# ZhengmaoHe/PARC

Hardware: AMD Instinct MI355X
Metric: env-steps/sec (whole node), 4096 envs/GPU humanoid tracker at 1/2/4/8 MI355X (higher is better)
Workload: dtype f32; 1 GPU; 4096 envs/GPU tracker on procgen box heightfields, 64 synthetic clips (BASELINE.json configs[2]); envs_per_gpu=4096, env_steps_per_bench_step=131072, rollout_steps=32, update_epochs=5, minibatch=16384, sim_substeps=4, parallelism=dp1, scaling_rule=per-rank work fixed (T = 32, minibatch = 4 x envs): weak scaling, grad_allreduce=per minibatch (reference cadence)

## Files before the change

include/parc_hip.h:

```cpp
#ifndef PARC_HIP_H
#define PARC_HIP_H

#include <stdint.h>

#ifdef __cplusplus
extern "C" {
#endif

#define PARC_MAX_BODIES 16
#define PARC_MAX_DOFS 64
#define PARC_MAX_TAR_STEPS 6
#define PARC_MAX_KEY_BODIES 8

#define PARC_OK 0
#define PARC_EINVAL (-1)
#define PARC_EUNSUPPORTED (-2)

#define PARC_JOINT_ROOT 0
#define PARC_JOINT_HINGE 1
#define PARC_JOINT_SPHERICAL 2
#define PARC_JOINT_FIXED 3

#define PARC_DONE_NULL 0
#define PARC_DONE_FAIL 1
// ... 199 lines not shown

int64_t parc_moments_workspace_floats(int64_t rows, int dim);
int parc_moments_accumulate(void *stream, int64_t rows, int dim, const float *x, float *acc, float *workspace);
int parc_obs_ingest(void *stream, int64_t rows, int dim, const float *x, const float *mean, const float *stdv, float clip, float *norm_out,
                    float *copy_dst, const int64_t *copy_row, float *acc, float *workspace);

int parc_action_head(void *stream, int n, int A, const float *mean, const float *logstd, const float *noise, const float *explore,
                     const float *a_mean, const float *a_std, float *action, float *logp);
int parc_action_head_record(void *stream, int n, int A, const float *mean, const float *logstd, const float *noise, const float *explore,
                            const float *a_mean, const float *a_std, float *action, float *logp, float *rec_action, float *rec_logp,
                            float *rec_mask, const float *forces_src, float *rec_forces, int n_forces, const int64_t *head);

int parc_points_hf_sdf(void *stream, int batch, int n_points, int dim_x, int dim_y, const float *points, const float *hf,
                       const float *min_box_center, const float *x_points, const float *y_points, float half_x, float half_y,
                       float base_z, int inverted, float radius, float *out, int32_t *out_cell);

int parc_points_hf_sdf_grad(void *stream, int batch, int n_points, int dim_x, int dim_y, const float *points, const float *hf,
                            const float *min_box_center, const float *x_points, const float *y_points, float half_x, float half_y,
                            float base_z, int inverted, const int32_t *cell, const float *g_out, float *g_points);

int64_t parc_relu_bwd_workspace_floats(int64_t rows, int dim);
int parc_relu_bwd_bias_grad(void *stream, int64_t rows, int dim, float *gy, const float *y, float *db, float *workspace);
int parc_weighted_colsum(void *stream, int64_t rows, int dim, const float *x, const float *w, float *out, float *workspace);

int parc_abi_version(void);

#ifdef __cplusplus
}
#endif
#endif
```

parc_amd/_hip.py:

```python
import ctypes
import os
import subprocess

import torch

_HERE = os.path.dirname(os.path.abspath(__file__))
LIB_DIR = os.path.join(_HERE, "lib")
LIB_PATH = os.path.join(LIB_DIR, "libparc_hip.so")
CSRC = os.path.join(_HERE, "csrc")
SOURCES = ["parc_kin.hip", "parc_sim.hip", "parc_ppo.hip", "parc_terrain.hip", "parc_render.hip", "parc_score.hip", "parc_netstats.hip", "parc_moopt.hip"]
DIAG_LIB_PATH = os.path.join(LIB_DIR, "libparc_hip_diag.so")
DIAG_SOURCES = SOURCES + ["parc_sim_ref.hip"]

MAX_BODIES = 16
MAX_DOFS = 64
MAX_TAR_STEPS = 6
MAX_KEY_BODIES = 8

POST_REF = 1
POST_OBS = 2
POST_REWARD_DONE = 4
POST_HF = 8
POST_MASKED = 16
POST_INIT_CHAR = 32
# ... 175 lines not shown
    L.parc_ppo_workspace_floats.restype = c_int
    L.parc_normalize_clamp.argtypes = [c_vp, c_i64, c_int, c_vp, c_vp, c_vp, c_f, c_vp]
    L.parc_normalize_clamp.restype = c_int
    L.parc_action_head.argtypes = [c_vp, c_int, c_int] + [c_vp] * 8
    L.parc_action_head.restype = c_int
    L.parc_action_head_record.argtypes = [c_vp, c_int, c_int] + [c_vp] * 8 + [c_vp] * 5 + [c_int, c_vp]
    L.parc_action_head_record.restype = c_int
    L.parc_points_hf_sdf.argtypes = [c_vp, c_int, c_int, c_int, c_int] + [c_vp] * 5 + [c_f, c_f, c_f, c_int, c_f, c_vp, c_vp]
    L.parc_points_hf_sdf.restype = c_int
    L.parc_points_hf_sdf_grad.argtypes = [c_vp, c_int, c_int, c_int, c_int] + [c_vp] * 5 + [c_f, c_f, c_f, c_int, c_vp, c_vp, c_vp]
    L.parc_points_hf_sdf_grad.restype = c_int
    L.parc_scale_by_clipped_norm.argtypes = [c_vp, c_i64, c_vp, c_vp, c_f]
    L.parc_scale_by_clipped_norm.restype = c_int
    L.parc_moments_workspace_floats.argtypes = [c_i64, c_int]
    L.parc_moments_workspace_floats.restype = c_i64
    L.parc_moments_accumulate.argtypes = [c_vp, c_i64, c_int, c_vp, c_vp, c_vp]
    L.parc_moments_accumulate.restype = c_int
    L.parc_relu_bwd_workspace_floats.argtypes = [c_i64, c_int]
    L.parc_relu_bwd_workspace_floats.restype = c_i64
    L.parc_relu_bwd_bias_grad.argtypes = [c_vp, c_i64, c_int, c_vp, c_vp, c_vp, c_vp]
    L.parc_relu_bwd_bias_grad.restype = c_int
    L.parc_weighted_colsum.argtypes = [c_vp, c_i64, c_int, c_vp, c_vp, c_vp, c_vp]
    L.parc_weighted_colsum.restype = c_int
    L.parc_sgd_workspace_floats.argtypes = []
    L.parc_sgd_workspace_floats.restype = c_i64
    L.parc_sgd_momentum_step.argtypes = [c_vp, c_i64, c_vp, c_vp, c_vp, c_f, c_f, c_f, c_f, c_vp, c_vp]
    L.parc_sgd_momentum_step.restype = c_int
    L.parc_adamw_step.argtypes = [c_vp, c_i64, c_vp, c_vp, c_vp, c_vp, c_i64, c_f, c_f, c_f, c_f, c_f, c_f, c_vp, c_vp]
    L.parc_adamw_step.restype = c_int
    L.parc_return_tracker_update.argtypes = [c_vp, c_int, c_int, c_vp, c_i64] + [c_vp] * 8
    L.parc_return_tracker_workspace_floats.argtypes = [c_int]
    L.parc_return_tracker_workspace_floats.restype = c_i64
    L.parc_return_tracker_update.restype = c_int
    L.parc_record_step.argtypes = [c_vp, c_int, c_vp, c_int, c_vp]
    L.parc_record_step.restype = c_int
    L.parc_obs_ingest.argtypes = [c_vp, c_i64, c_int, c_vp, c_vp, c_vp, c_f, c_vp, c_vp, c_vp, c_vp, c_vp]
    L.parc_obs_ingest.restype = c_int
    L.parc_rng_step.argtypes = [c_vp, ctypes.c_uint64, c_vp, c_vp, c_i64, c_vp, c_i64, c_vp, c_int]
    L.parc_rng_step.restype = c_int
    L.parc_reset_apply.argtypes = [c_vp, c_int, c_vp, c_vp, c_vp, c_vp, c_vp, c_int] + [c_vp] * 9
    L.parc_reset_apply.restype = c_int
    L.parc_reset_sample_apply.argtypes = [c_vp, c_int, c_vp, c_vp, c_vp, c_int, c_vp, c_vp, c_f, c_vp, c_vp, c_int, c_f] + [c_vp] * 11
    L.parc_reset_sample_apply.restype = c_int
    for name in ("parc_refresh_ray_obs_hfs", "parc_refresh_obs_hfs", "parc_dof_to_rot", "parc_rot_to_dof",
                 "parc_forward_kinematics", "parc_calc_motion_frame", "parc_motion_lib_build", "parc_track_post_step", "parc_reset_apply",
                 "parc_update_fail_rates", "parc_td_lambda_return", "parc_adv_normalize"):
# ... 6 lines not shown
        _hip_render.declare(L)
    if hasattr(L, "parc_score_abi"):
        from . import _hip_score
        _hip_score.declare(L)
    if hasattr(L, "parc_netstats_abi"):
        from . import _hip_netstats
        _hip_netstats.declare(L)
    if hasattr(L, "parc_moopt_abi"):
        from . import _hip_moopt
        _hip_moopt.declare(L)


EXPORTED = ["parc_abi_version", "parc_refresh_ray_obs_hfs", "parc_refresh_obs_hfs", "parc_dof_to_rot", "parc_rot_to_dof",
            "parc_forward_kinematics", "parc_calc_motion_frame", "parc_motion_lib_build", "parc_track_post_step",
            "parc_update_fail_rates", "parc_td_lambda_return", "parc_adv_normalize", "parc_reset_apply", "parc_ppo_loss", "parc_ppo_workspace_floats", "parc_record_step", "parc_return_tracker_update", "parc_normalize_clamp",
            "parc_action_head", "parc_points_hf_sdf", "parc_moments_workspace_floats", "parc_moments_accumulate", "parc_reset_sample_apply", "parc_return_tracker_workspace_floats", "parc_scale_by_clipped_norm", "parc_relu_bwd_workspace_floats",
            "parc_relu_bwd_bias_grad", "parc_ppo_loss_packed", "parc_weighted_colsum", "parc_sgd_workspace_floats", "parc_sgd_momentum_step", "parc_adamw_step",
            "parc_pose_chain_forward", "parc_pose_chain_backward", "parc_points_hf_sdf_grad", "parc_body_points_world", "parc_body_points_world_grad",
            "parc_quat_diff_angle", "parc_quat_diff_angle_grad", "parc_temporal_terms", "parc_temporal_terms_grad", "parc_step_tail",
            "parc_assemble_obs", "parc_track_post_step_timed", "parc_rng_step", "parc_obs_ingest", "parc_action_head_record",
            "parc_render", "parc_render_abi", "parc_motion_score", "parc_score_abi",
            "parc_netstats_workspace_floats", "parc_netstats_update", "parc_netstats_abs_colsum", "parc_netstats_dormant_count", "parc_netstats_abi",
            "parc_points_hf_sdf_ragged", "parc_points_hf_sdf_ragged_grad", "parc_temporal_terms_seg", "parc_temporal_terms_seg_grad",
            "parc_segment_sums", "parc_moopt_abi"]


def check(rc, what):
    if rc != 0:
        raise RuntimeError("{} failed with code {} ({})".format(what, rc, "bad argument" if rc == -1 else "unsupported" if rc == -2 else "hipError"))


def stream():
    return c_vp(torch.cuda.current_stream().cuda_stream)


def ptr(t):
    if t is None:
        return c_vp(0)
    assert t.is_cuda, "HIP kernels need device tensors (no CPU fallback)"
    assert t.is_contiguous(), "tensor must be contiguous"
    return c_vp(t.data_ptr())


def terrain_struct(hf, min_point, dxdy):
    assert hf.dtype == torch.float32 and hf.is_contiguous() and hf.dim() == 2
    return TerrainS(ptr(hf), int(hf.shape[0]), int(hf.shape[1]), float(min_point[0]), float(min_point[1]),
                    float(dxdy[0]), float(dxdy[1]))
# ... 29 lines not shown
```

parc_amd/csrc/parc_ppo.hip:

```cpp
#include <hip/hip_runtime.h>
#include <math.h>
#include <stdint.h>
#include <stdio.h>
#include <stdlib.h>

#include "../../include/parc_hip.h"

#define PPO_THREADS 256
#define PPO_MAX_A 64
#define PPO_NSCAL 8
#define PPO_W (PPO_NSCAL + PPO_MAX_A)

__device__ __forceinline__ float wave_sum(float v) {
#pragma unroll
    for (int o = 32; o >= 1; o >>= 1) v += __shfl_xor(v, o, 64);
    return v;
}

__device__ __forceinline__ float clamp_nan(float v, float lo, float hi) { return v < lo ? lo : (v > hi ? hi : v); }
__device__ __forceinline__ float clamp_min_nan(float v, float lo) { return v < lo ? lo : v; }
__device__ __forceinline__ float clamp_max_nan(float v, float hi) { return v > hi ? hi : v; }
__device__ __forceinline__ float minimum_nan(float a, float b) { return a <= b ? a : (b < a ? b : __builtin_nanf("")); }
__device__ __forceinline__ float clip_coef(float max_norm, float norm) { return clamp_max_nan(max_norm / (norm + 1e-6f), 1.0f); }

// ... 184 lines not shown
        out[0] = actor_loss + cfg.critic_w * critic_loss;
        out[1] = critic_loss;
        out[2] = actor_loss;
        out[3] = s[3] / cnt;
        out[4] = s[4] / cnt;
        out[5] = abl;
        out[6] = ent;
        out[7] = regl;
        out[8] = cnt;
        out[9] = gate / cnt;
        out[10] = cfg.critic_w / (float)B;
    }
}

__global__ __launch_bounds__(256) void ppo_scale_kernel(int n_mean, int n_pred, const float *__restrict__ out, float *g_mean, float *g_pred) {
    const int i = blockIdx.x * blockDim.x + threadIdx.x;
    const float sa = out[9], sp = out[10];
    if (i < n_mean) g_mean[i] *= sa;
    if (i < n_pred) g_pred[i] *= sp;
}

static int ppo_loss_impl(void *stream, int B, int A, const float *mean, const float *logstd, const float *norm_a, const float *old_logp,
                         const float *adv, const float *mask, const float *pred, const float *tar_val, parc_ppo_cfg_t cfg, float *g_mean,
                         float *g_logstd, float *g_pred, float *out, float *workspace, int a_stride, int s_stride);

extern "C" int parc_ppo_loss(void *stream, int B, int A, const float *mean, const float *logstd, const float *norm_a, const float *old_logp,
                             const float *adv, const float *mask, const float *pred, const float *tar_val, parc_ppo_cfg_t cfg, float *g_mean,
                             float *g_logstd, float *g_pred, float *out, float *workspace) {
    return ppo_loss_impl(stream, B, A, mean, logstd, norm_a, old_logp, adv, mask, pred, tar_val, cfg, g_mean, g_logstd, g_pred, out, workspace, A, 1);
}

extern "C" int parc_ppo_loss_packed(void *stream, int B, int A, const float *mean, const float *logstd, const float *rec, int rec_stride,
                                    const float *pred, parc_ppo_cfg_t cfg, float *g_mean, float *g_logstd, float *g_pred, float *out,
                                    float *workspace) {
    if (!rec || rec_stride < A + 4) return PARC_EINVAL;
    return ppo_loss_impl(stream, B, A, mean, logstd, rec, rec + A, rec + A + 1, rec + A + 2, pred, rec + A + 3, cfg, g_mean, g_logstd, g_pred, out,
                         workspace, rec_stride, rec_stride);
}

static int ppo_loss_impl(void *stream, int B, int A, const float *mean, const float *logstd, const float *norm_a, const float *old_logp,
                         const float *adv, const float *mask, const float *pred, const float *tar_val, parc_ppo_cfg_t cfg, float *g_mean,
                         float *g_logstd, float *g_pred, float *out, float *workspace, int a_stride, int s_stride) {
    if (B <= 0 || A <= 0 || A > PPO_MAX_A) return PARC_EINVAL;
    int nblk = (B + PPO_THREADS - 1) / PPO_THREADS;
    hipStream_t st = (hipStream_t)stream;
    if (A <= 32) {
        nblk = (B + PPO32_SPB - 1) / PPO32_SPB;
        hipLaunchKernelGGL(ppo_sample32_kernel, dim3(nblk), dim3(256), 0, st, B, A, mean, logstd, norm_a, old_logp, adv, mask, pred, tar_val, cfg,
                           g_mean, g_pred, workspace, a_stride, s_stride);
    } else {
        hipLaunchKernelGGL(ppo_sample_kernel, dim3(nblk), dim3(PPO_THREADS), 0, st, B, A, mean, logstd, norm_a, old_logp, adv, mask, pred, tar_val,
                           cfg, g_mean, g_pred, workspace, a_stride, s_stride);
    }
    hipLaunchKernelGGL(ppo_reduce_kernel, dim3(1), dim3(PPO_RED_THREADS), 0, st, B, A, nblk, logstd, cfg, workspace, g_logstd, out);
    const int n = B * A;
    hipLaunchKernelGGL(ppo_scale_kernel, dim3((n + 255) / 256), dim3(256), 0, st, n, B, out, g_mean, g_pred);
    hipError_t e = hipGetLastError();
    return e == hipSuccess ? PARC_OK : (int)e;
}

extern "C" int parc_ppo_workspace_floats(int B) { return ((B + PPO32_SPB - 1) / PPO32_SPB) * PPO_W; }

#define PARC_RECORD_MAX_FIELDS 12
struct record_fields_t {
    parc_record_field_t f[PARC_RECORD_MAX_FIELDS];
};

__global__ __launch_bounds__(256) void record_step_kernel(int n_envs, const int64_t *__restrict__ head, record_fields_t fields) {
    const parc_record_field_t f = fields.f[blockIdx.y];
    const size_t total = (size_t)n_envs * (size_t)f.row_bytes;
    const size_t h = (size_t)head[0];
    const size_t tid = (size_t)blockIdx.x * blockDim.x + threadIdx.x, nthr = (size_t)gridDim.x * blockDim.x;
    if (f.convert == 1) {
        const int64_t *s = (const int64_t *)f.src;
        int32_t *d = (int32_t *)f.dst + h * (total / 8);
        for (size_t i = tid; i < total / 8; i += nthr) d[i] = (int32_t)s[i];
        return;
    }
    if (f.convert == 2) {
// ... 574 lines not shown
    hipLaunchKernelGGL(colsum_final_kernel, dim3((dim + 255) / 256), dim3(256), 0, (hipStream_t)stream, chunks, dim, workspace, out);
    hipError_t e = hipGetLastError();
    return e == hipSuccess ? PARC_OK : (int)e;
}

extern "C" int64_t parc_relu_bwd_workspace_floats(int64_t rows, int dim) {
    if (rows < 0 || dim <= 0) return -1;
    return ((rows + RB_ROWS - 1) / RB_ROWS) * (int64_t)dim;
}

extern "C" int parc_relu_bwd_bias_grad(void *stream, int64_t rows, int dim, float *gy, const float *y, float *db, float *workspace) {
    if (rows < 0 || dim <= 0 || (dim & 3) || !gy || !y || !db || !workspace || (((uintptr_t)gy | (uintptr_t)y | (uintptr_t)workspace) & 15))
        return PARC_EINVAL;
    if (rows > (int64_t)RB_ROWS * 65535) return PARC_EUNSUPPORTED;
    const int dim4 = dim / 4, chunks = (int)((rows + RB_ROWS - 1) / RB_ROWS);
    if (rows > 0)
        hipLaunchKernelGGL(relu_bwd_bias_partial_kernel, dim3((dim4 + 63) / 64, chunks), dim3(256), 0, (hipStream_t)stream, (int)rows, dim4,
                           (float4 *)gy, (const float4 *)y, (float4 *)workspace);
    hipLaunchKernelGGL(colsum_final_kernel, dim3((dim + 255) / 256), dim3(256), 0, (hipStream_t)stream, chunks, dim, workspace, db);
    hipError_t e = hipGetLastError();
    return e == hipSuccess ? PARC_OK : (int)e;
}

__global__ __launch_bounds__(256) void action_head_kernel(int n, int A, const float *__restrict__ mean, const float *__restrict__ logstd,
                                                          const float *__restrict__ noise, const float *__restrict__ explore,
                                                          const float *__restrict__ a_mean, const float *__restrict__ a_std, float *action,
                                                          float *logp) {
    const int i = blockIdx.x * blockDim.x + threadIdx.x;
    if (i >= n) return;
    const bool ex = explore[i] == 1.0f;
    float acc = 0.f, sum_ls = 0.f;
    for (int j = 0; j < A; ++j) {
        const float ls = logstd[j], sd = __expf(ls);
        const float mu = mean[(size_t)i * A + j];
        const float na = ex ? mu + sd * noise[(size_t)i * A + j] : mu;
        const float z = (na - mu) / sd;
        acc = fmaf(z, z, acc);
        sum_ls += ls;
        action[(size_t)i * A + j] = na * a_std[j] + a_mean[j];
    }
    logp[i] = -0.5f * acc + (-0.5f * (float)A * 1.8378770664093453f - sum_ls);
}

struct action_record_t {
    float *action, *logp, *mask, *forces;
    const float *forces_src;
// ... 73 lines not shown
```

parc_amd/learning/dm_ppo_agent.py:

```python
import enum
import os
import time

import numpy as np
import torch

from ..envs import base_env
from ..gym_spaces import Box
from ..util import mp_util
from ..util.logger import Logger
from . import dm_ppo_model, experience_buffer, mp_optimizer, normalizer, rl_util, unit_stats
from .dm_ppo_return_tracker import DMPPOReturnTracker
from .tracking_error_tracker import TrackingErrorTracker


class AgentMode(enum.Enum):
    TRAIN = 0
    TEST = 1


_LOSS_KEYS = ["norm_obs", "action", "a_logp", "tar_val", "adv", "rand_action_mask"]


def enable_tuned_gemms():
# ... 466 lines not shown
                        "test_mean_body_rot_tracking_err": t.get_mean_body_rot_err().item(),
                        "test_mean_dof_vel_tracking_err": t.get_mean_dof_vel_err().item(),
                        "test_mean_root_vel_tracking_err": t.get_mean_root_vel_err().item(),
                        "test_mean_root_ang_vel_tracking_err": t.get_mean_root_ang_vel_err().item()})
        return out

    def hard_reset_envs(self):
        if self._is_terrain_runner:
            self._env.apply_hard_reset()
        self._curr_obs, self._curr_info = self._env.reset()

    def test_model(self, num_episodes):
        self.eval()
        self.set_mode(AgentMode.TEST)
        self.hard_reset_envs()
        P = mp_util.get_num_procs()
        return self._rollout_test(int(np.ceil(num_episodes / P)))

    @torch.no_grad()
    def _critic_values(self):
        eb = self._exp_buffer
        obs, next_obs, done = eb.get_data("obs"), eb.get_data("next_obs"), eb.get_data("done")
        norm_obs = self._obs_norm.normalize(obs, out=eb.get_data("norm_obs"))
        vals = self._model.eval_critic(norm_obs).squeeze(-1)
        T = obs.shape[0]
        need = done != base_env.DoneFlags.NULL.value
        need[T - 1] = True
        next_vals = torch.empty_like(vals)
        next_vals[:T - 1] = vals[1:]
        idx = need.flatten().nonzero().flatten()
        sel = next_obs.flatten(0, 1)[idx]
        next_vals.flatten()[idx] = self._model.eval_critic(self._obs_norm.normalize(sel)).squeeze(-1)
        return vals, next_vals

    @torch.no_grad()
    def _build_train_data(self):
        self.eval()
        eb = self._exp_buffer
        obs, next_obs = eb.get_data("obs"), eb.get_data("next_obs")
        r, done = eb.get_data("reward"), eb.get_data("done")
        mask = eb.get_data("rand_action_mask")
        vals, next_vals = self._critic_values()
        r_min, r_max = self._env.get_reward_bounds()
        next_vals = torch.clamp(next_vals, r_min / (1.0 - self._discount), r_max / (1.0 - self._discount))
        succ_val = self._env.get_reward_succ() / (1.0 - self._discount)
        fail_val = self._env.get_reward_fail() / (1.0 - self._discount)
        next_vals = torch.where(done == base_env.DoneFlags.SUCC.value, torch.full_like(next_vals, succ_val), next_vals)
        next_vals = torch.where(done == base_env.DoneFlags.FAIL.value, torch.full_like(next_vals, fail_val), next_vals)
# ... 60 lines not shown
            return None
        loss, out = rl_util.ppo_loss(a_dist.mean, logstd[0], pred, norm_a, batch["a_logp"], batch["adv"], batch["rand_action_mask"],
                                     batch["tar_val"], self._ppo_clip_ratio, self._action_bound_weight, self._action_entropy_weight,
                                     self._action_reg_weight, self._critic_loss_weight, 20.0, self._critic_loss_type != "L2")
        slots = {"loss": 0, "critic_loss": 1, "actor_loss": 2, "clip_frac": 3, "imp_ratio": 4}
        if self._action_bound_weight != 0:
            slots["action_bound_loss"] = 5
        if self._action_entropy_weight != 0:
            slots["action_entropy"] = 6
        if self._action_reg_weight != 0:
            slots["action_reg_loss"] = 7
        return {"loss": loss, "_packed": out, "_slots": slots}

    def _explicit_update_ok(self):
        return (str(self._device).startswith("cuda") and self._config.get("explicit_backward", True) and self._config.get("fused_ppo_loss", True)
                and self._model.supports_explicit_backward())

    def _minibatch_step_explicit(self, batch, acc):
        norm_obs = batch["norm_obs"]
        mean, logstd, pred, saved = self._model.train_forward(norm_obs)
        if self._ppo_cfg is None:
            self._ppo_cfg = rl_util.ppo_cfg(self._ppo_clip_ratio, self._action_bound_weight, self._action_entropy_weight, self._action_reg_weight,
                                            self._critic_loss_weight, 20.0, self._critic_loss_type != "L2")
        if "loss_rec" in batch:
            out, g_mean, g_logstd, g_pred = rl_util.ppo_loss_and_grads_packed(mean, logstd, pred, batch["loss_rec"], self._ppo_cfg)
        else:
            out, g_mean, g_logstd, g_pred = rl_util.ppo_loss_and_grads(mean, logstd, pred, self._a_norm.normalize(batch["action"]), batch["a_logp"],
                                                                        batch["adv"], batch["rand_action_mask"], batch["tar_val"], self._ppo_cfg)
        write = lambda grad_of, done: self._model.train_backward(saved, g_mean, g_logstd, g_pred, grad_of, done)
        if self._clip_grad_norm:
            self._optimizer.step_explicit(write, model=self._model, max_norm=self._max_grad_norm)
        else:
            self._optimizer.step_explicit(write)
        acc.append(out)

    def _nan_trap(self, loss_rows, batches, epoch):
        bad = torch.isnan(loss_rows).any(dim=1).tolist()
        if not any(bad):
            return
        k = bad.index(True)
        import pickle
        batch_file = os.path.join("output", "debug_batch.pkl")
        os.makedirs("output", exist_ok=True)
        with open(batch_file, "wb") as f:
            pickle.dump({name: v.detach().cpu() for name, v in batches[k].items()}, f)
        Logger.print("NAN LOSS in minibatch {} of update epoch {}: wrote debug batch file to {}".format(k, epoch, batch_file))
        raise FloatingPointError("NaN loss in minibatch {} of update epoch {} (batch dumped to {}; the reference prints, dumps and exits "
                                 "at this point)".format(k, epoch, batch_file))

    def _update_model(self):
        self.train()
        N = self.get_num_envs()
# ... 196 lines not shown
```

parc_amd/learning/dm_ppo_model.py:

```python
import enum

import numpy as np
import torch


class StdType(enum.Enum):
    FIXED = 0
    CONSTANT = 1
    VARIABLE = 2


class DistributionGaussianDiag:
    def __init__(self, mean, logstd):
        self._mean = mean
        self._logstd = logstd
        self._std_cache = None
        self._dim = mean.shape[-1]

    @property
    def _std(self):
        if self._std_cache is None:
            self._std_cache = torch.exp(self._logstd)
        return self._std_cache

# ... 156 lines not shown
        pred = torch.addmm(self._critic_out.bias, c[-1], self._critic_out.weight.t()).squeeze(-1)
        return mean, self._action_dist._logstd_net, pred, (a, c)

    def _relu_bwd(self, d, y, db):
        from .. import _hip
        L = _hip.lib()
        need = int(L.parc_relu_bwd_workspace_floats(d.shape[0], d.shape[1]))
        ws = getattr(self, "_relu_ws", None)
        if ws is None or ws.numel() < need or ws.device != d.device:
            ws = self._relu_ws = torch.empty(max(need, 1), dtype=torch.float32, device=d.device)
        _hip.check(L.parc_relu_bwd_bias_grad(_hip.stream(), d.shape[0], d.shape[1], _hip.ptr(d), _hip.ptr(y), _hip.ptr(db), _hip.ptr(ws)),
                   "parc_relu_bwd_bias_grad")

    def _weighted_colsum(self, x, w, out):
        from .. import _hip
        L = _hip.lib()
        need = int(L.parc_relu_bwd_workspace_floats(x.shape[0], x.shape[1]))
        ws = getattr(self, "_relu_ws", None)
        if ws is None or ws.numel() < need or ws.device != x.device:
            ws = self._relu_ws = torch.empty(max(need, 1), dtype=torch.float32, device=x.device)
        _hip.check(L.parc_weighted_colsum(_hip.stream(), x.shape[0], x.shape[1], _hip.ptr(x), _hip.ptr(w.contiguous()), _hip.ptr(out), _hip.ptr(ws)),
                   "parc_weighted_colsum")

    def _trunk_backward(self, seq, acts, d, grad_of, done):
        lins = list(seq)[0::2]
        for k in range(len(lins) - 1, -1, -1):
            lin = lins[k]
            self._relu_bwd(d, acts[k + 1], grad_of(lin.bias))
            torch.mm(d.t(), acts[k], out=grad_of(lin.weight))
            done(lin.weight)
            done(lin.bias)
            if k > 0:
                d = torch.mm(d, lin.weight)

    @torch.no_grad()
    def train_backward(self, saved, g_mean, g_logstd, g_pred, grad_of, done=lambda p: None):
        a, c = saved
        mnet = self._action_dist._mean_net
        torch.mm(g_mean.t(), a[-1], out=grad_of(mnet.weight))
        torch.sum(g_mean, dim=0, out=grad_of(mnet.bias))
        done(mnet.weight)
        done(mnet.bias)
        if self._action_dist._std_type == StdType.CONSTANT:
            grad_of(self._action_dist._logstd_net).copy_(g_logstd)
            done(self._action_dist._logstd_net)
        self._trunk_backward(self._actor_layers, a, torch.mm(g_mean, mnet.weight), grad_of, done)
        gp = g_pred.unsqueeze(-1)
        if self._critic_out.weight.shape[0] == 1:
            self._weighted_colsum(c[-1], g_pred, grad_of(self._critic_out.weight).view(-1))
        else:
            torch.mm(gp.t(), c[-1], out=grad_of(self._critic_out.weight))
        torch.sum(gp, dim=0, out=grad_of(self._critic_out.bias))
        done(self._critic_out.weight)
        done(self._critic_out.bias)
        self._trunk_backward(self._critic_layers, c, torch.mm(gp, self._critic_out.weight), grad_of, done)

    def eval_critic(self, obs):
        return self._critic_out(self._critic_layers(obs))
```

parc_amd/learning/rl_util.py:

```python
import torch

from .. import _hip

_workspace = {}


def compute_td_lambda_return(r, next_vals, done, discount, td_lambda):
    assert r.shape == next_vals.shape and r.dim() == 2
    r = r.contiguous().float()
    nv = next_vals.contiguous().float()
    dn = done.contiguous().to(torch.int32)
    T, N = r.shape
    ret = torch.empty_like(r)
    _hip.check(_hip.lib().parc_td_lambda_return(_hip.stream(), T, N, _hip.ptr(r), _hip.ptr(nv), _hip.ptr(dn), float(discount),
                                                float(td_lambda), _hip.ptr(ret)), "parc_td_lambda_return")
    return ret


def normalize_advantage(ret, vals, rand_action_mask, clip):
    ret = ret.contiguous().float()
    vals = vals.contiguous().float()
    mask = rand_action_mask.contiguous().float()
    dev = ret.device
    ws = _workspace.get(dev)
    if ws is None:
        ws = torch.empty(3 * 1024, dtype=torch.float64, device=dev)
        _workspace[dev] = ws
    out = torch.empty_like(ret)
    ms = torch.empty(2, dtype=torch.float32, device=dev)
    _hip.check(_hip.lib().parc_adv_normalize(_hip.stream(), ret.numel(), _hip.ptr(ret), _hip.ptr(vals), _hip.ptr(mask), float(clip),
                                             _hip.ptr(out), _hip.ptr(ms), _hip.ptr(ws)), "parc_adv_normalize")
    return out, ms


def ppo_loss_and_grads(mean, logstd, pred, norm_a, old_logp, adv, mask, tar_val, cfg):
    from .. import _hip
    B, A = mean.shape
    mean, norm_a = mean.contiguous(), norm_a.contiguous()
    g_mean = torch.empty_like(mean)
    g_logstd = torch.empty_like(logstd)
    g_pred = torch.empty(B, dtype=torch.float32, device=mean.device)
    out = torch.empty(16, dtype=torch.float32, device=mean.device)
    ws = torch.empty(_hip.lib().parc_ppo_workspace_floats(B), dtype=torch.float32, device=mean.device)
    p = _hip.ptr
    _hip.check(_hip.lib().parc_ppo_loss(_hip.stream(), B, A, p(mean), p(logstd.contiguous()), p(norm_a), p(old_logp.contiguous()),
                                        p(adv.contiguous()), p(mask.contiguous()), p(pred.contiguous()), p(tar_val.contiguous()), cfg,
                                        p(g_mean), p(g_logstd), p(g_pred), p(out), p(ws)), "parc_ppo_loss")
    return out, g_mean, g_logstd, g_pred


def ppo_loss_and_grads_packed(mean, logstd, pred, rec, cfg):
    from .. import _hip
    B, A = mean.shape
    assert rec.dim() == 2 and rec.shape[0] == B and rec.shape[1] >= A + 4 and rec.is_contiguous()
    mean = mean.contiguous()
    g_mean = torch.empty_like(mean)
    g_logstd = torch.empty_like(logstd)
    g_pred = torch.empty(B, dtype=torch.float32, device=mean.device)
    out = torch.empty(16, dtype=torch.float32, device=mean.device)
    ws = torch.empty(_hip.lib().parc_ppo_workspace_floats(B), dtype=torch.float32, device=mean.device)
    p = _hip.ptr
    _hip.check(_hip.lib().parc_ppo_loss_packed(_hip.stream(), B, A, p(mean), p(logstd.contiguous()), p(rec), int(rec.shape[1]), p(pred.contiguous()),
                                               cfg, p(g_mean), p(g_logstd), p(g_pred), p(out), p(ws)), "parc_ppo_loss_packed")
    return out, g_mean, g_logstd, g_pred


def ppo_cfg(clip_ratio, bound_w, entropy_w, reg_w, critic_w, large_critic_loss=20.0, critic_l1=False):
    from .. import _hip
    return _hip.PPOCfgS(float(clip_ratio), float(bound_w), float(entropy_w), float(reg_w), float(critic_w), float(large_critic_loss),
                        int(bool(critic_l1)))


class _PPOLossFn(torch.autograd.Function):

    @staticmethod
    def forward(ctx, mean, logstd, pred, norm_a, old_logp, adv, mask, tar_val, cfg):
        out, g_mean, g_logstd, g_pred = ppo_loss_and_grads(mean, logstd, pred, norm_a, old_logp, adv, mask, tar_val, cfg)
        ctx.save_for_backward(g_mean, g_logstd, g_pred)
        ctx.mark_non_differentiable(out)
        return out[0], out

    @staticmethod
    def backward(ctx, g_loss, _g_out):
        g_mean, g_logstd, g_pred = ctx.saved_tensors
        return g_mean * g_loss, g_logstd * g_loss, g_pred * g_loss, None, None, None, None, None, None

# ... 6 lines not shown
```

Measured before the change: 454,400 env-steps/s.

## Fuse output-head backward with ReLU mask, bias and weight gradients

Adds a HIP head-backward kernel that computes the output-layer weight and bias gradients, the propagated gradient through the head weights, the ReLU mask, and the last hidden layer's bias gradient in one pass over the activations. The default critic path (J=1) now uses it instead of separate weighted-colsum, matmul and relu-bwd launches. An optional mode skips the PPO loss scale kernel and folds the loss scales into the head backward, but it is disabled by default. The aim is fewer kernel launches and fewer reads of the large activation tensor in the minibatch backward. The cost is extra code paths and a reduction order that differs from before.

```diff
diff --git a/include/parc_hip.h b/include/parc_hip.h
--- a/include/parc_hip.h
+++ b/include/parc_hip.h
@@ -245,6 +245,15 @@
 int64_t parc_relu_bwd_workspace_floats(int64_t rows, int dim);
 int parc_relu_bwd_bias_grad(void *stream, int64_t rows, int dim, float *gy, const float *y, float *db, float *workspace);
 int parc_weighted_colsum(void *stream, int64_t rows, int dim, const float *x, const float *w, float *out, float *workspace);
+int64_t parc_head_bwd_workspace_floats(int64_t rows, int h, int J);
+int parc_head_bwd(void *stream, int64_t rows, int h, int J, const float *Wh, const float *g, const float *scale, const float *y, float *d,
+                  float *db, float *dWh, float *dbh, float *workspace);
+int parc_ppo_loss_unscaled(void *stream, int B, int A, const float *mean, const float *logstd, const float *norm_a, const float *old_logp,
+                           const float *adv, const float *mask, const float *pred, const float *tar_val, parc_ppo_cfg_t cfg, float *g_mean,
+                           float *g_logstd, float *g_pred, float *out, float *workspace);
+int parc_ppo_loss_packed_unscaled(void *stream, int B, int A, const float *mean, const float *logstd, const float *rec, int rec_stride,
+                                  const float *pred, parc_ppo_cfg_t cfg, float *g_mean, float *g_logstd, float *g_pred, float *out,
+                                  float *workspace);
 
 int parc_abi_version(void);
 
diff --git a/parc_amd/_hip.py b/parc_amd/_hip.py
--- a/parc_amd/_hip.py
+++ b/parc_amd/_hip.py
@@ -221,6 +221,14 @@
     L.parc_relu_bwd_bias_grad.restype = c_int
     L.parc_weighted_colsum.argtypes = [c_vp, c_i64, c_int, c_vp, c_vp, c_vp, c_vp]
     L.parc_weighted_colsum.restype = c_int
+    L.parc_head_bwd_workspace_floats.argtypes = [c_i64, c_int, c_int]
+    L.parc_head_bwd_workspace_floats.restype = c_i64
+    L.parc_head_bwd.argtypes = [c_vp, c_i64, c_int, c_int] + [c_vp] * 9
+    L.parc_head_bwd.restype = c_int
+    L.parc_ppo_loss_unscaled.argtypes = L.parc_ppo_loss.argtypes
+    L.parc_ppo_loss_unscaled.restype = c_int
+    L.parc_ppo_loss_packed_unscaled.argtypes = L.parc_ppo_loss_packed.argtypes
+    L.parc_ppo_loss_packed_unscaled.restype = c_int
     L.parc_sgd_workspace_floats.argtypes = []
     L.parc_sgd_workspace_floats.restype = c_i64
     L.parc_sgd_momentum_step.argtypes = [c_vp, c_i64, c_vp, c_vp, c_vp, c_f, c_f, c_f, c_f, c_vp, c_vp]
@@ -273,7 +281,8 @@
             "parc_render", "parc_render_abi", "parc_motion_score", "parc_score_abi",
             "parc_netstats_workspace_floats", "parc_netstats_update", "parc_netstats_abs_colsum", "parc_netstats_dormant_count", "parc_netstats_abi",
             "parc_points_hf_sdf_ragged", "parc_points_hf_sdf_ragged_grad", "parc_temporal_terms_seg", "parc_temporal_terms_seg_grad",
-            "parc_segment_sums", "parc_moopt_abi"]
+            "parc_segment_sums", "parc_moopt_abi",
+            "parc_head_bwd_workspace_floats", "parc_head_bwd", "parc_ppo_loss_unscaled", "parc_ppo_loss_packed_unscaled"]
 
 
 def check(rc, what):
diff --git a/parc_amd/csrc/parc_ppo.hip b/parc_amd/csrc/parc_ppo.hip
--- a/parc_amd/csrc/parc_ppo.hip
+++ b/parc_amd/csrc/parc_ppo.hip
@@ -230,7 +230,7 @@
 
 static int ppo_loss_impl(void *stream, int B, int A, const float *mean, const float *logstd, const float *norm_a, const float *old_logp,
                          const float *adv, const float *mask, const float *pred, const float *tar_val, parc_ppo_cfg_t cfg, float *g_mean,
-                         float *g_logstd, float *g_pred, float *out, float *workspace, int a_stride, int s_stride);
+                         float *g_logstd, float *g_pred, float *out, float *workspace, int a_stride, int s_stride, bool apply_scale = true);
 
 extern "C" int parc_ppo_loss(void *stream, int B, int A, const float *mean, const float *logstd, const float *norm_a, const float *old_logp,
                              const float *adv, const float *mask, const float *pred, const float *tar_val, parc_ppo_cfg_t cfg, float *g_mean,
@@ -246,9 +246,24 @@
                          workspace, rec_stride, rec_stride);
 }
 
+extern "C" int parc_ppo_loss_unscaled(void *stream, int B, int A, const float *mean, const float *logstd, const float *norm_a, const float *old_logp,
+                                      const float *adv, const float *mask, const float *pred, const float *tar_val, parc_ppo_cfg_t cfg,
+                                      float *g_mean, float *g_logstd, float *g_pred, float *out, float *workspace) {
+    return ppo_loss_impl(stream, B, A, mean, logstd, norm_a, old_logp, adv, mask, pred, tar_val, cfg, g_mean, g_logstd, g_pred, out, workspace, A, 1,
+                         false);
+}
+
+extern "C" int parc_ppo_loss_packed_unscaled(void *stream, int B, int A, const float *mean, const float *logstd, const float *rec, int rec_stride,
+                                             const float *pred, parc_ppo_cfg_t cfg, float *g_mean, float *g_logstd, float *g_pred, float *out,
+                                             float *workspace) {
+    if (!rec || rec_stride < A + 4) return PARC_EINVAL;
+    return ppo_loss_impl(stream, B, A, mean, logstd, rec, rec + A, rec + A + 1, rec + A + 2, pred, rec + A + 3, cfg, g_mean, g_logstd, g_pred, out,
+                         workspace, rec_stride, rec_stride, false);
+}
+
 static int ppo_loss_impl(void *stream, int B, int A, const float *mean, const float *logstd, const float *norm_a, const float *old_logp,
                          const float *adv, const float *mask, const float *pred, const float *tar_val, parc_ppo_cfg_t cfg, float *g_mean,
-                         float *g_logstd, float *g_pred, float *out, float *workspace, int a_stride, int s_stride) {
+                         float *g_logstd, float *g_pred, float *out, float *workspace, int a_stride, int s_stride, bool apply_scale) {
     if (B <= 0 || A <= 0 || A > PPO_MAX_A) return PARC_EINVAL;
     int nblk = (B + PPO_THREADS - 1) / PPO_THREADS;
     hipStream_t st = (hipStream_t)stream;
@@ -262,7 +277,7 @@
     }
     hipLaunchKernelGGL(ppo_reduce_kernel, dim3(1), dim3(PPO_RED_THREADS), 0, st, B, A, nblk, logstd, cfg, workspace, g_logstd, out);
     const int n = B * A;
-    hipLaunchKernelGGL(ppo_scale_kernel, dim3((n + 255) / 256), dim3(256), 0, st, n, B, out, g_mean, g_pred);
+    if (apply_scale) hipLaunchKernelGGL(ppo_scale_kernel, dim3((n + 255) / 256), dim3(256), 0, st, n, B, out, g_mean, g_pred);
     hipError_t e = hipGetLastError();
     return e == hipSuccess ? PARC_OK : (int)e;
 }
@@ -883,6 +898,256 @@
     return e == hipSuccess ? PARC_OK : (int)e;
 }
 
+#define HB_ROWS 64
+#define HB_COLS 512
+template <int JP, int NS>
+__global__ __launch_bounds__(256 * NS) void head_bwd_partial_kernel(int rows, int h, int J, const float *__restrict__ Wh, const float *__restrict__ g,
+                                                                    const float *__restrict__ scale, const float *__restrict__ y,
+                                                                    float *__restrict__ d, float *__restrict__ partial) {
+    constexpr int HB_U = JP >= 16 ? 4 : 8;
+    constexpr int GR = HB_ROWS / NS;
+    constexpr int NV = 2 * JP + 2;
+    __shared__ __attribute__((aligned(16))) float s_g[HB_ROWS * JP];
+    __shared__ float s_fold[(NS - 1) * NV * 256];
+    const int tid = threadIdx.x & 255, grp = threadIdx.x >> 8;
+    const int r0 = blockIdx.y * HB_ROWS, nr = min(HB_ROWS, rows - r0);
+    const int c0 = blockIdx.x * HB_COLS + tid, c1 = c0 + 256;
+    const bool v0 = c0 < h, v1 = c1 < h;
+    const int cc0 = v0 ? c0 : 0, cc1 = v1 ? c1 : 0;
+    const float sc = scale ? scale[0] : 1.f;
+    for (int i = threadIdx.x; i < HB_ROWS * JP; i += 256 * NS) {
+        const int r = i / JP, j = i - r * JP;
+        float v = 0.f;
+        if (r < nr && j < J) {
+            v = g[(size_t)(r0 + r) * J + j];
+            if (scale) v *= sc;
+        }
+        s_g[i] = v;
+    }
+    float w0[JP], w1[JP], a0[JP], a1[JP];
+#pragma unroll
+    for (int j = 0; j < JP; ++j) {
+        w0[j] = j < J ? Wh[(size_t)j * h + cc0] : 0.f;
+        w1[j] = j < J ? Wh[(size_t)j * h + cc1] : 0.f;
+        a0[j] = 0.f;
+        a1[j] = 0.f;
+    }
+    float b0 = 0.f, b1 = 0.f;
+    const int g0 = grp * GR, ge = min(g0 + GR, nr);
+    const float *yb = y + (size_t)r0 * h;
+    float *dr = d + (size_t)r0 * h;
+    float n0[HB_U], n1[HB_U];
+#pragma unroll
+    for (int u = 0; u < HB_U; ++u) {
+        const int r = min(g0 + u, nr - 1);
+        n0[u] = yb[(size_t)r * h + cc0];
+        n1[u] = yb[(size_t)r * h + cc1];
+    }
+    __syncthreads();
+    for (int rb = g0; rb < ge; rb += HB_U) {
+        float y0[HB_U], y1[HB_U];
+#pragma unroll
+        for (int u = 0; u < HB_U; ++u) {
+            y0[u] = n0[u];
+            y1[u] = n1[u];
+        }
+#pragma unroll
+        for (int u = 0; u < HB_U; ++u) {
+            const int r = min(rb + HB_U + u, nr - 1);
+            n0[u] = yb[(size_t)r * h + cc0];
+            n1[u] = yb[(size_t)r * h + cc1];
+        }
+#pragma unroll
+        for (int u = 0; u < HB_U; ++u) {
+            const int r = rb + u;
+            if (r < ge) {
+                const float *gr = s_g + r * JP;
+                float s0 = 0.f, s1 = 0.f;
+#pragma unroll
+                for (int j = 0; j < JP; ++j) {
+                    const float gj = gr[j];
+                    s0 = fmaf(gj, w0[j], s0);
+                    s1 = fmaf(gj, w1[j], s1);
+                    a0[j] = fmaf(gj, y0[u], a0[j]);
+                    a1[j] = fmaf(gj, y1[u], a1[j]);
+                }
+                const float d0 = y0[u] <= 0.f ? 0.f : s0, d1 = y1[u] <= 0.f ? 0.f : s1;
+                if (v0) dr[(size_t)r * h + c0] = d0;
+                if (v1) dr[(size_t)r * h + c1] = d1;
+                b0 += d0;
+                b1 += d1;
+            }
+        }
+    }
+    if (grp > 0) {
+        float *f = s_fold + (size_t)(grp - 1) * NV * 256 + tid;
+#pragma unroll
+        for (int j = 0; j < JP; ++j) {
+            f[(2 * j) * 256] = a0[j];
+            f[(2 * j + 1) * 256] = a1[j];
+        }
+        f[(2 * JP) * 256] = b0;
+        f[(2 * JP + 1) * 256] = b1;
+    }
+    __syncthreads();
+    if (grp > 0) return;
+#pragma unroll
+    for (int s = 0; s < NS - 1; ++s) {
+        const float *f = s_fold + (size_t)s * NV * 256 + tid;
+#pragma unroll
+        for (int j = 0; j < JP; ++j) {
+            a0[j] += f[(2 * j) * 256];
+            a1[j] += f[(2 * j + 1) * 256];
+        }
+        b0 += f[(2 * JP) * 256];
+        b1 += f[(2 * JP + 1) * 256];
+    }
+    float *p = partial + (size_t)blockIdx.y * ((size_t)J * h + h + J);
+#pragma unroll
+    for (int j = 0; j < JP; ++j) {
+        if (j < J) {
+            if (v0) p[(size_t)j * h + c0] = a0[j];
+            if (v1) p[(size_t)j * h + c1] = a1[j];
+        }
+    }
+    if (v0) p[(size_t)J * h + c0] = b0;
+    if (v1) p[(size_t)J * h + c1] = b1;
+    if (blockIdx.x == 0 && tid < J) {
+        float t = 0.f;
+        for (int r = 0; r < nr; ++r) t += s_g[r * JP + tid];
+        p[(size_t)J * h + h + tid] = t;
+    }
+}
+
+template <int P>
+__global__ __launch_bounds__(256) void head_bwd_final_kernel(int chunks, int h, int J, const float *__restrict__ partial, float *__restrict__ dWh,
+                                                             float *__restrict__ db, float *__restrict__ dbh) {
+    constexpr int E = 256 / P;
+    __shared__ float sp[P][E];
+    const int lane = threadIdx.x % E, part = threadIdx.x / E;
+    const int n = J * h + h + J, e = blockIdx.x * E + lane;
+    const int per = (chunks + P - 1) / P, k0 = part * per, k1 = min(k0 + per, chunks);
+    float t = 0.f;
+    if (e < n) {
+#pragma unroll 16
+        for (int k = k0; k < k1; ++k) t += partial[(size_t)k * n + e];
+    }
+    sp[part][lane] = t;
+    __syncthreads();
+    if (part == 0 && e < n) {
+        float v = sp[0][lane];
+#pragma unroll
+        for (int q = 1; q < P; ++q) v += sp[q][lane];
+        if (e < J * h) dWh[e] = v;
+        else if (e < J * h + h) db[e - J * h] = v;
+        else dbh[e - J * h - h] = v;
+    }
+}
+
+__global__ __launch_bounds__(256) void head1_bwd_partial_kernel(int rows, int dim4, const float4 *__restrict__ wh, const float *__restrict__ g,
+                                                                const float *__restrict__ scale, const float4 *__restrict__ y,
+                                                                float4 *__restrict__ d, float4 *__restrict__ partial, float *__restrict__ pbh) {
+    __shared__ float4 red[2][4][64];
+    const int lane = threadIdx.x & 63, rg = threadIdx.x >> 6;
+    const int c = blockIdx.x * 64 + lane;
+    const int r0 = blockIdx.y * RB_ROWS, r1 = min(r0 + RB_ROWS, rows);
+    const float sc = scale ? scale[0] : 1.f;
+    float4 s = make_float4(0.f, 0.f, 0.f, 0.f), t = s;
+    if (c < dim4) {
+        const float4 w = wh[c];
+#pragma unroll 4
+        for (int r = r0 + rg; r < r1; r += 4) {
+            const size_t i = (size_t)r * dim4 + c;
+            const float4 v = y[i];
+            float gr = g[r];
+            if (scale) gr *= sc;
+            s.x = fmaf(gr, v.x, s.x); s.y = fmaf(gr, v.y, s.y); s.z = fmaf(gr, v.z, s.z); s.w = fmaf(gr, v.w, s.w);
+            float4 o;
+            o.x = v.x <= 0.f ? 0.f : __fmul_rn(gr, w.x); o.y = v.y <= 0.f ? 0.f : __fmul_rn(gr, w.y);
+            o.z = v.z <= 0.f ? 0.f : __fmul_rn(gr, w.z); o.w = v.w <= 0.f ? 0.f : __fmul_rn(gr, w.w);
+            d[i] = o;
+            t.x += o.x; t.y += o.y; t.z += o.z; t.w += o.w;
+        }
+    }
+    red[0][rg][lane] = s;
+    red[1][rg][lane] = t;
+    __syncthreads();
+    if (rg < 2 && c < dim4) {
+        const float4 a = red[rg][0][lane], b = red[rg][1][lane], e = red[rg][2][lane], f = red[rg][3][lane];
+        float4 o;
+        o.x = (a.x + b.x) + (e.x + f.x); o.y = (a.y + b.y) + (e.y + f.y); o.z = (a.z + b.z) + (e.z + f.z); o.w = (a.w + b.w) + (e.w + f.w);
+        partial[((size_t)blockIdx.y * 2 + rg) * dim4 + c] = o;
+    }
+    if (pbh && blockIdx.x == 0 && threadIdx.x == 0) {
+        float b = 0.f;
+        for (int r = r0; r < r1; ++r) {
+            float gr = g[r];
+            if (scale) gr *= sc;
+            b += gr;
+        }
+        pbh[blockIdx.y] = b;
+    }
+}
+
+__global__ __launch_bounds__(256) void head1_bwd_final_kernel(int chunks, int dim, const float *__restrict__ partial, const float *__restrict__ pbh,
+                                                              float *__restrict__ dWh, float *__restrict__ db, float *__restrict__ dbh) {
+    const int e = blockIdx.x * blockDim.x + threadIdx.x;
+    if (e > 2 * dim || (e == 2 * dim && !dbh)) return;
+    float t = 0.f;
+    if (e == 2 * dim) {
+        for (int k = 0; k < chunks; ++k) t += pbh[k];
+        dbh[0] = t;
+        return;
+    }
+    const int which = e / dim, c = e - which * dim;
+#pragma unroll 16
+    for (int k = 0; k < chunks; ++k) t += partial[((size_t)k * 2 + which) * dim + c];
+    (which ? db : dWh)[c] = t;
+}
+
+extern "C" int64_t parc_head_bwd_workspace_floats(int64_t rows, int h, int J) {
+    if (rows < 0 || h <= 0 || J <= 0) return -1;
+    return ((rows + HB_ROWS - 1) / HB_ROWS) * ((int64_t)J * h + h + J);
+}
+
+extern "C" int parc_head_bwd(void *stream, int64_t rows, int h, int J, const float *Wh, const float *g, const float *scale, const float *y, float *d,
+                             float *db, float *dWh, float *dbh, float *workspace) {
+    if (rows < 0 || h <= 0 || (h & 3) || J < 1 || J > 32 || !Wh || !g || !y || !d || !db || !dWh || (!dbh && J > 1) || !workspace) return PARC_EINVAL;
+    if (rows > (int64_t)HB_ROWS * 65535 || h > (1 << 22)) return PARC_EUNSUPPORTED;
+    hipStream_t st = (hipStream_t)stream;
+    if (J == 1 && !(((uintptr_t)Wh | (uintptr_t)y | (uintptr_t)d | (uintptr_t)workspace) & 15)) {
+        const int dim4 = h / 4, ch = (int)((rows + RB_ROWS - 1) / RB_ROWS);
+        float *pbh = workspace + (size_t)ch * 2 * h;
+        if (rows > 0)
+            hipLaunchKernelGGL(head1_bwd_partial_kernel, dim3((dim4 + 63) / 64, ch), dim3(256), 0, st, (int)rows, dim4, (const float4 *)Wh, g, scale,
+                               (const float4 *)y, (float4 *)d, (float4 *)workspace, dbh ? pbh : (float *)nullptr);
+        hipLaunchKernelGGL(head1_bwd_final_kernel, dim3((2 * h + 1 + 255) / 256), dim3(256), 0, st, ch, h, workspace, pbh, dWh, db, dbh);
+        hipError_t e1 = hipGetLastError();
+        return e1 == hipSuccess ? PARC_OK : (int)e1;
+    }
+    if (!dbh) return PARC_EINVAL;
+    const int chunks = (int)((rows + HB_ROWS - 1) / HB_ROWS);
+    if (rows > 0) {
+        const dim3 grid((h + HB_COLS - 1) / HB_COLS, chunks);
+#define HB_LAUNCH(JP, NS) \
+    hipLaunchKernelGGL((head_bwd_partial_kernel<JP, NS>), grid, dim3(256 * NS), 0, st, (int)rows, h, J, Wh, g, scale, y, d, workspace)
+        if (J == 1) HB_LAUNCH(1, 4);
+        else if (J <= 4) HB_LAUNCH(4, 4);
+        else if (J <= 8) HB_LAUNCH(8, 4);
+        else if (J <= 16) HB_LAUNCH(16, 2);
+        else if (J <= 28) HB_LAUNCH(28, 2);
+        else HB_LAUNCH(32, 2);
+#undef HB_LAUNCH
+    }
+    const int n = J * h + h + J;
+    if (n >= 8192)
+        hipLaunchKernelGGL(head_bwd_final_kernel<4>, dim3((n + 63) / 64), dim3(256), 0, st, chunks, h, J, workspace, dWh, db, dbh);
+    else
+        hipLaunchKernelGGL(head_bwd_final_kernel<16>, dim3((n + 15) / 16), dim3(256), 0, st, chunks, h, J, workspace, dWh, db, dbh);
+    hipError_t e = hipGetLastError();
+    return e == hipSuccess ? PARC_OK : (int)e;
+}
+
 __global__ __launch_bounds__(256) void action_head_kernel(int n, int A, const float *__restrict__ mean, const float *__restrict__ logstd,
                                                           const float *__restrict__ noise, const float *__restrict__ explore,
                                                           const float *__restrict__ a_mean, const float *__restrict__ a_std, float *action,
diff --git a/parc_amd/learning/dm_ppo_agent.py b/parc_amd/learning/dm_ppo_agent.py
--- a/parc_amd/learning/dm_ppo_agent.py
+++ b/parc_amd/learning/dm_ppo_agent.py
@@ -512,8 +512,13 @@
         eb = self._exp_buffer
         obs, next_obs, done = eb.get_data("obs"), eb.get_data("next_obs"), eb.get_data("done")
         norm_obs = self._obs_norm.normalize(obs, out=eb.get_data("norm_obs"))
-        vals = self._model.eval_critic(norm_obs).squeeze(-1)
-        T = obs.shape[0]
+        T, N = obs.shape[:2]
+        rows = norm_obs.reshape(T * N, -1)
+        vals = torch.empty(T, N, dtype=torch.float32, device=rows.device)
+        flat_vals = vals.view(-1, 1)
+        block = max(int(self._batch_size * N), 1)
+        for r0 in range(0, T * N, block):
+            flat_vals[r0:r0 + block] = self._model.eval_critic(rows[r0:r0 + block])
         need = done != base_env.DoneFlags.NULL.value
         need[T - 1] = True
         next_vals = torch.empty_like(vals)
@@ -620,12 +625,17 @@
         if self._ppo_cfg is None:
             self._ppo_cfg = rl_util.ppo_cfg(self._ppo_clip_ratio, self._action_bound_weight, self._action_entropy_weight, self._action_reg_weight,
                                             self._critic_loss_weight, 20.0, self._critic_loss_type != "L2")
+        self._model.fused_heads = bool(self._config.get("fused_heads", True))
+        self._model.fused_policy_head = bool(self._config.get("fused_policy_head", False))
+        fused = self._model.heads_take_unscaled_grads(saved)
         if "loss_rec" in batch:
-            out, g_mean, g_logstd, g_pred = rl_util.ppo_loss_and_grads_packed(mean, logstd, pred, batch["loss_rec"], self._ppo_cfg)
+            out, g_mean, g_logstd, g_pred = rl_util.ppo_loss_and_grads_packed(mean, logstd, pred, batch["loss_rec"], self._ppo_cfg, apply_scale=not fused)
         else:
             out, g_mean, g_logstd, g_pred = rl_util.ppo_loss_and_grads(mean, logstd, pred, self._a_norm.normalize(batch["action"]), batch["a_logp"],
-                                                                        batch["adv"], batch["rand_action_mask"], batch["tar_val"], self._ppo_cfg)
-        write = lambda grad_of, done: self._model.train_backward(saved, g_mean, g_logstd, g_pred, grad_of, done)
+                                                                        batch["adv"], batch["rand_action_mask"], batch["tar_val"], self._ppo_cfg,
+                                                                        apply_scale=not fused)
+        scales = (out[9:10], out[10:11]) if fused else None
+        write = lambda grad_of, done: self._model.train_backward(saved, g_mean, g_logstd, g_pred, grad_of, done, scales=scales)
         if self._clip_grad_norm:
             self._optimizer.step_explicit(write, model=self._model, max_norm=self._max_grad_norm)
         else:
diff --git a/parc_amd/learning/dm_ppo_model.py b/parc_amd/learning/dm_ppo_model.py
--- a/parc_amd/learning/dm_ppo_model.py
+++ b/parc_amd/learning/dm_ppo_model.py
@@ -202,11 +202,38 @@
         _hip.check(L.parc_weighted_colsum(_hip.stream(), x.shape[0], x.shape[1], _hip.ptr(x), _hip.ptr(w.contiguous()), _hip.ptr(out), _hip.ptr(ws)),
                    "parc_weighted_colsum")
 
-    def _trunk_backward(self, seq, acts, d, grad_of, done):
+    fused_heads = True
+    fused_policy_head = False
+
+    def _head_bwd_ok(self, head, y):
+        return (self.fused_heads and y.is_cuda and head.out_features <= 32 and y.shape[1] % 4 == 0
+                and self._action_dist._std_type != StdType.VARIABLE)
+
+    def heads_take_unscaled_grads(self, saved):
+        a, c = saved
+        return bool(self.fused_policy_head) and self._head_bwd_ok(self._action_dist._mean_net, a[-1]) and self._head_bwd_ok(self._critic_out, c[-1])
+
+    def _head_bwd(self, head, g, scale, y, grad_of, db, bias_grad=True):
+        from .. import _hip
+        L = _hip.lib()
+        B, h = y.shape
+        J = head.out_features
+        need = int(L.parc_head_bwd_workspace_floats(B, h, J))
+        ws = getattr(self, "_relu_ws", None)
+        if ws is None or ws.numel() < need or ws.device != y.device:
+            ws = self._relu_ws = torch.empty(max(need, 1), dtype=torch.float32, device=y.device)
+        d = torch.empty_like(y)
+        p = _hip.ptr
+        _hip.check(L.parc_head_bwd(_hip.stream(), B, h, J, p(head.weight), p(g.contiguous()), p(scale), p(y), p(d), p(db), p(grad_of(head.weight)),
+                                   p(grad_of(head.bias) if bias_grad else None), p(ws)), "parc_head_bwd")
+        return d
+
+    def _trunk_backward(self, seq, acts, d, grad_of, done, last_masked=False):
         lins = list(seq)[0::2]
         for k in range(len(lins) - 1, -1, -1):
             lin = lins[k]
-            self._relu_bwd(d, acts[k + 1], grad_of(lin.bias))
+            if not (last_masked and k == len(lins) - 1):
+                self._relu_bwd(d, acts[k + 1], grad_of(lin.bias))
             torch.mm(d.t(), acts[k], out=grad_of(lin.weight))
             done(lin.weight)
             done(lin.bias)
@@ -214,9 +241,26 @@
                 d = torch.mm(d, lin.weight)
 
     @torch.no_grad()
-    def train_backward(self, saved, g_mean, g_logstd, g_pred, grad_of, done=lambda p: None):
+    def train_backward(self, saved, g_mean, g_logstd, g_pred, grad_of, done=lambda p: None, scales=None):
         a, c = saved
         mnet = self._action_dist._mean_net
+        s_mean, s_pred = scales if scales is not None else (None, None)
+        if self.heads_take_unscaled_grads(saved):
+            last = list(self._actor_layers)[-2]
+            d = self._head_bwd(mnet, g_mean, s_mean, a[-1], grad_of, grad_of(last.bias))
+            done(mnet.weight)
+            done(mnet.bias)
+            if self._action_dist._std_type == StdType.CONSTANT:
+                grad_of(self._action_dist._logstd_net).copy_(g_logstd)
+                done(self._action_dist._logstd_net)
+            self._trunk_backward(self._actor_layers, a, d, grad_of, done, last_masked=True)
+            last = list(self._critic_layers)[-2]
+            d = self._head_bwd(self._critic_out, g_pred, s_pred, c[-1], grad_of, grad_of(last.bias))
+            done(self._critic_out.weight)
+            done(self._critic_out.bias)
+            self._trunk_backward(self._critic_layers, c, d, grad_of, done, last_masked=True)
+            return
+        assert scales is None, "unscaled output gradients need both heads on the fused backward"
         torch.mm(g_mean.t(), a[-1], out=grad_of(mnet.weight))
         torch.sum(g_mean, dim=0, out=grad_of(mnet.bias))
         done(mnet.weight)
@@ -226,6 +270,14 @@
             done(self._action_dist._logstd_net)
         self._trunk_backward(self._actor_layers, a, torch.mm(g_mean, mnet.weight), grad_of, done)
         gp = g_pred.unsqueeze(-1)
+        if self._critic_out.weight.shape[0] == 1 and self._head_bwd_ok(self._critic_out, c[-1]) and self._critic_out.weight.data_ptr() % 16 == 0:
+            last = list(self._critic_layers)[-2]
+            d = self._head_bwd(self._critic_out, g_pred, None, c[-1], grad_of, grad_of(last.bias), bias_grad=False)
+            torch.sum(gp, dim=0, out=grad_of(self._critic_out.bias))
+            done(self._critic_out.weight)
+            done(self._critic_out.bias)
+            self._trunk_backward(self._critic_layers, c, d, grad_of, done, last_masked=True)
+            return
         if self._critic_out.weight.shape[0] == 1:
             self._weighted_colsum(c[-1], g_pred, grad_of(self._critic_out.weight).view(-1))
         else:
diff --git a/parc_amd/learning/rl_util.py b/parc_amd/learning/rl_util.py
--- a/parc_amd/learning/rl_util.py
+++ b/parc_amd/learning/rl_util.py
@@ -33,7 +33,7 @@
     return out, ms
 
 
-def ppo_loss_and_grads(mean, logstd, pred, norm_a, old_logp, adv, mask, tar_val, cfg):
+def ppo_loss_and_grads(mean, logstd, pred, norm_a, old_logp, adv, mask, tar_val, cfg, apply_scale=True):
     from .. import _hip
     B, A = mean.shape
     mean, norm_a = mean.contiguous(), norm_a.contiguous()
@@ -43,13 +43,14 @@
     out = torch.empty(16, dtype=torch.float32, device=mean.device)
     ws = torch.empty(_hip.lib().parc_ppo_workspace_floats(B), dtype=torch.float32, device=mean.device)
     p = _hip.ptr
-    _hip.check(_hip.lib().parc_ppo_loss(_hip.stream(), B, A, p(mean), p(logstd.contiguous()), p(norm_a), p(old_logp.contiguous()),
-                                        p(adv.contiguous()), p(mask.contiguous()), p(pred.contiguous()), p(tar_val.contiguous()), cfg,
-                                        p(g_mean), p(g_logstd), p(g_pred), p(out), p(ws)), "parc_ppo_loss")
+    fn = _hip.lib().parc_ppo_loss if apply_scale else _hip.lib().parc_ppo_loss_unscaled
+    _hip.check(fn(_hip.stream(), B, A, p(mean), p(logstd.contiguous()), p(norm_a), p(old_logp.contiguous()),
+                  p(adv.contiguous()), p(mask.contiguous()), p(pred.contiguous()), p(tar_val.contiguous()), cfg,
+                  p(g_mean), p(g_logstd), p(g_pred), p(out), p(ws)), "parc_ppo_loss")
     return out, g_mean, g_logstd, g_pred
 
 
-def ppo_loss_and_grads_packed(mean, logstd, pred, rec, cfg):
+def ppo_loss_and_grads_packed(mean, logstd, pred, rec, cfg, apply_scale=True):
     from .. import _hip
     B, A = mean.shape
     assert rec.dim() == 2 and rec.shape[0] == B and rec.shape[1] >= A + 4 and rec.is_contiguous()
@@ -60,8 +61,9 @@
     out = torch.empty(16, dtype=torch.float32, device=mean.device)
     ws = torch.empty(_hip.lib().parc_ppo_workspace_floats(B), dtype=torch.float32, device=mean.device)
     p = _hip.ptr
-    _hip.check(_hip.lib().parc_ppo_loss_packed(_hip.stream(), B, A, p(mean), p(logstd.contiguous()), p(rec), int(rec.shape[1]), p(pred.contiguous()),
-                                               cfg, p(g_mean), p(g_logstd), p(g_pred), p(out), p(ws)), "parc_ppo_loss_packed")
+    fn = _hip.lib().parc_ppo_loss_packed if apply_scale else _hip.lib().parc_ppo_loss_packed_unscaled
+    _hip.check(fn(_hip.stream(), B, A, p(mean), p(logstd.contiguous()), p(rec), int(rec.shape[1]), p(pred.contiguous()),
+                  cfg, p(g_mean), p(g_logstd), p(g_pred), p(out), p(ws)), "parc_ppo_loss_packed")
     return out, g_mean, g_logstd, g_pred
 
 
```

Result: no change. 457,500 env-steps/s (median of 6 runs) (+0.7%).
